# claudiotomasi/LearnMultigrid

Hardware: NVIDIA B200
Metric: vcycle_fine_grid_dof_per_s (higher is better)
Workload: dtype f64

## Files before the change

### include/mgb200.h

```cpp
#ifndef MGB200_H
#define MGB200_H

#include <stdint.h>

#ifdef __cplusplus
extern "C" {
#endif

typedef enum {
    MG_OK = 0,
    MG_ERR_INVALID = -1,
    MG_ERR_CUDA = -2,
    MG_ERR_UNSUPPORTED = -3,
    MG_ERR_OVERFLOW = -4,
    MG_ERR_SINGULAR = -5
} mg_status;

int mg_version(void);
const char *mg_last_error(void);
int64_t mg_struct_size(int which);
int mg_set_pdl(int enabled);
int mg_device_info(int *sm_count, int64_t *global_mem, int *cc);


// ... 11 lines not shown
int mg_gs_lex_sweep_csr(int64_t n, const int32_t *d_indptr, const int32_t *d_indices, const double *d_values,
                        double *d_x, const double *d_b, const int64_t *d_level_ptr,
                        const int32_t *d_level_rows, int64_t nlevels, int iterations, void *stream);
int mg_prolong_correct_csr(int64_t n, const int32_t *d_indptr, const int32_t *d_indices,
                           const double *d_values, const double *d_e, double *d_u, void *stream);

typedef struct {
    int64_t nrows;
    int64_t ncols;
    int64_t nslices;
    const int64_t *d_slice_ptr;
    const int32_t *d_cols;
    const double *d_vals;
    int64_t max_slice_len;
    int64_t uniform_len;
    const uint16_t *d_slice_rec;
    const int32_t *d_rec_table;
    int32_t nrec, n_spec;
    const int64_t *h_spec_row;
    const int32_t *h_spec_rec;
    const unsigned char *d_val_idx;
    const double *d_val_table;
    const double *d_rec_vals;
    const double *h_spec_vals;
} mg_sell;

int mg_sell_slice_offsets(const mg_sell *A, int32_t *d_off, int64_t *d_nregular, void *stream);
int64_t mg_value_dict_workspace(void);
int mg_value_dict_build(int64_t n, const double *d_vals, unsigned char *d_index, double *d_table, void *d_work,
                        int *h_count, void *stream);
int mg_set_value_dict(int enabled);
int mg_set_implied_values(int enabled);
int mg_set_implied_columns(int enabled);
int64_t mg_set_implied_min_rows(int64_t rows);
int mg_sell_spmv(const mg_sell *A, const double *d_x, double *d_y, void *stream);
int mg_sell_residual(const mg_sell *A, const double *d_x, const double *d_b, double *d_r, void *stream);
int mg_sell_residual_rows(const mg_sell *A, const double *d_x, const double *d_b, double *d_r, int64_t row0,
                          int64_t row1, void *stream);
int mg_sell_residual_norm2(const mg_sell *A, const double *d_x, const double *d_b, double *d_partials,
                           double *d_norm2, void *stream);
int64_t mg_norm_workspace_size(int64_t n);
int64_t mg_set_tma_min_rows(int64_t rows);
int64_t mg_set_wide_min_len(int64_t len);
int mg_set_short_rows_per_thread(int r);
int64_t mg_set_short_min_rows(int64_t rows);
int64_t mg_set_wide_max_rows(int64_t rows);
int mg_sell_jacobi(const mg_sell *A, const double *d_dinv, const double *d_x, const double *d_b,
                   double *d_x_out, double omega, void *stream);
int mg_sell_gs_rows(const mg_sell *A, double *d_x, const double *d_b, int64_t row0, int64_t row1,
                    void *stream);
int mg_sell_gs_rows_tail(const mg_sell *A, double *d_x, const double *d_b, int64_t row0, int64_t row1, int tail,
                         double *d_r, double *d_partials, int *h_nblocks, void *stream);
int mg_sell_gs_tail_ok(const mg_sell *A, int64_t row0, int64_t row1);
int mg_sell_gs_zero_first(int64_t n_vec, int64_t row0, int64_t row1, const double *d_diag, const double *d_b,
                          double *d_x, void *stream);
int mg_sell_prolong_correct(const mg_sell *Q, const double *d_e, const double *d_u, double *d_u_out,
                            void *stream);
int mg_sell_prolong_correct_rows(const mg_sell *Q, const double *d_e, const double *d_u, double *d_u_out, int64_t row0,
                                 int64_t row1, void *stream);

int mg_dot(int64_t n, const double *d_x, const double *d_y, double *d_partials, double *d_out, void *stream);
int mg_axpby(int64_t n, double a, const double *d_x, double b, const double *d_y, double *d_out, void *stream);
int mg_fill(int64_t n, double value, double *d_x, void *stream);
int mg_gather(int64_t n, const int32_t *d_idx, const double *d_in, double *d_out, void *stream);
int mg_scatter(int64_t n, const int32_t *d_idx, const double *d_in, double *d_out, void *stream);

// ... 270 lines not shown
```

### learnmultigrid_b200/_lib.py

```python
import ctypes
import os
import subprocess

_HERE = os.path.dirname(os.path.abspath(__file__))
LIB_PATH = os.path.join(_HERE, "libmgb200.so")
CSRC = os.path.join(_HERE, "csrc")

c_i32p = ctypes.c_void_p
c_f64p = ctypes.c_void_p
c_i64 = ctypes.c_int64
c_int = ctypes.c_int
c_dbl = ctypes.c_double
c_vp = ctypes.c_void_p

MG_SMOOTH_JACOBI, MG_SMOOTH_MCGS, MG_SMOOTH_LEXGS = 0, 1, 2
MG_COARSE_DENSE, MG_COARSE_BCR = 0, 1
MG_LEVEL_PROPER_COLORING, MG_LEVEL_NONZERO_DIAG = 1, 2
SLICE_IRREGULAR = -2 ** 31


class MgError(RuntimeError):
    pass


# ... 80 lines not shown
    "mg_device_info": (c_int, [ctypes.POINTER(c_int), ctypes.POINTER(c_i64), ctypes.POINTER(c_int)]),
    "mg_spmv_csr": (c_int, [c_i64, c_vp, c_vp, c_vp, c_vp, c_vp, c_vp]),
    "mg_residual_csr": (c_int, [c_i64, c_vp, c_vp, c_vp, c_vp, c_vp, c_vp, c_vp]),
    "mg_jacobi_sweep_csr": (c_int, [c_i64, c_vp, c_vp, c_vp, c_vp, c_vp, c_vp, c_vp, c_dbl, c_vp]),
    "mg_gs_multicolor_sweep_csr": (c_int, [c_i64, c_vp, c_vp, c_vp, c_vp, c_vp, ctypes.POINTER(c_i64), c_vp,
                                           c_int, c_vp]),
    "mg_gs_lex_sweep_csr": (c_int, [c_i64, c_vp, c_vp, c_vp, c_vp, c_vp, c_vp, c_vp, c_i64, c_int, c_vp]),
    "mg_prolong_correct_csr": (c_int, [c_i64, c_vp, c_vp, c_vp, c_vp, c_vp, c_vp]),
    "mg_sell_spmv": (c_int, [ctypes.POINTER(mg_sell), c_vp, c_vp, c_vp]),
    "mg_sell_slice_offsets": (c_int, [ctypes.POINTER(mg_sell), c_vp, c_vp, c_vp]),
    "mg_set_implied_min_rows": (c_i64, [c_i64]),
    "mg_tri_boxes_2d": (c_int, [c_i64, c_vp, c_vp, c_vp, c_vp, ctypes.c_int32, c_vp, c_vp, c_vp]),
    "mg_tri_incidence_2d": (c_int, [c_i64, c_vp, c_vp, c_vp, ctypes.c_int32, c_vp, c_vp, c_vp, c_vp]),
    "mg_tri_pairs_2d": (c_int, [c_i64, c_vp, c_vp, c_vp, c_vp, ctypes.c_int32, c_vp, c_vp, c_vp, c_vp, c_vp, c_vp, c_vp]),
    "mg_value_dict_workspace": (c_i64, []),
    "mg_value_dict_build": (c_int, [c_i64, c_vp, c_vp, c_vp, c_vp, ctypes.POINTER(c_int), c_vp]),
    "mg_set_value_dict": (c_int, [c_int]),
    "mg_set_implied_values": (c_int, [c_int]),
    "mg_set_short_rows_per_thread": (c_int, [c_int]),
    "mg_set_short_min_rows": (c_i64, [c_i64]),
    "mg_level_inspect": (c_int, [ctypes.POINTER(mg_sell), c_int, c_vp, c_vp, c_vp, c_vp]),
    "mg_sell_residual_rows": (c_int, [ctypes.POINTER(mg_sell), c_vp, c_vp, c_vp, c_i64, c_i64, c_vp]),
    "mg_sell_gs_rows_tail": (c_int, [ctypes.POINTER(mg_sell), c_vp, c_vp, c_i64, c_i64, c_int, c_vp, c_vp,
                                     ctypes.POINTER(c_int), c_vp]),
    "mg_sell_gs_tail_ok": (c_int, [ctypes.POINTER(mg_sell), c_i64, c_i64]),
    "mg_sell_gs_zero_first": (c_int, [c_i64, c_i64, c_i64, c_vp, c_vp, c_vp, c_vp]),
    "mg_sell_prolong_correct_rows": (c_int, [ctypes.POINTER(mg_sell), c_vp, c_vp, c_vp, c_i64, c_i64, c_vp]),
    "mg_vcycle_norm": (c_int, [ctypes.POINTER(mg_level), c_int, ctypes.POINTER(mg_cycle_params), c_vp, c_vp, c_vp]),
    "mg_set_cycle_fusion": (c_int, [c_int]),
    "mg_pcg_start": (c_int, [c_vp, ctypes.POINTER(mg_level), ctypes.POINTER(mg_pcg), c_vp]),
    "mg_pcg_iterate": (c_int, [c_vp, ctypes.POINTER(mg_level), c_int, ctypes.POINTER(mg_cycle_params),
                               ctypes.POINTER(mg_pcg), c_int, c_vp]),
    "mg_set_implied_columns": (c_int, [c_int]),
    "mg_sell_residual": (c_int, [ctypes.POINTER(mg_sell), c_vp, c_vp, c_vp, c_vp]),
    "mg_sell_residual_norm2": (c_int, [ctypes.POINTER(mg_sell), c_vp, c_vp, c_vp, c_vp, c_vp]),
    "mg_norm_workspace_size": (c_i64, [c_i64]),
    "mg_set_tma_min_rows": (c_i64, [c_i64]),
    "mg_sell_halo_mask": (c_int, [ctypes.POINTER(mg_sell), c_i64, c_vp, c_vp]),
    "mg_set_fused_exchange": (c_int, [c_int]),
    "mg_set_wide_min_len": (c_i64, [c_i64]),
    "mg_set_wide_max_rows": (c_i64, [c_i64]),
    "mg_sell_jacobi": (c_int, [ctypes.POINTER(mg_sell), c_vp, c_vp, c_vp, c_vp, c_dbl, c_vp]),
    "mg_sell_gs_rows": (c_int, [ctypes.POINTER(mg_sell), c_vp, c_vp, c_i64, c_i64, c_vp]),
    "mg_sell_prolong_correct": (c_int, [ctypes.POINTER(mg_sell), c_vp, c_vp, c_vp, c_vp]),
    "mg_dot": (c_int, [c_i64, c_vp, c_vp, c_vp, c_vp, c_vp]),
    "mg_axpby": (c_int, [c_i64, c_dbl, c_vp, c_dbl, c_vp, c_vp, c_vp]),
    "mg_fill": (c_int, [c_i64, c_dbl, c_vp, c_vp]),
    "mg_gather": (c_int, [c_i64, c_vp, c_vp, c_vp, c_vp]),
    "mg_scatter": (c_int, [c_i64, c_vp, c_vp, c_vp, c_vp]),
    "mg_dense_inverse": (c_int, [c_i64, c_vp, c_vp, c_vp, c_vp]),
    "mg_dense_inverse_workspace": (c_i64, [c_i64]),
    "mg_dense_gemv": (c_int, [c_i64, c_i64, c_vp, c_vp, c_vp, c_vp]),
    "mg_bcr_blocks_from_csr": (c_int, [c_i64, c_i64, c_i64, c_vp, c_vp, c_vp, c_vp, c_vp, c_vp, c_vp, c_vp]),
    "mg_dense_inverse_batched": (c_int, [c_i64, c_i64, c_vp, c_i64, c_vp, c_i64, c_vp, c_vp, c_vp]),
    "mg_dense_gemm_batched": (c_int, [c_i64, c_i64, c_vp, c_i64, c_vp, c_i64, c_vp, c_i64, c_dbl, c_dbl, c_vp]),
    "mg_bcr_solve": (c_int, [ctypes.POINTER(mg_bcr), c_vp, c_vp, c_vp]),
    "mg_bcr_solve_dist": (c_int, [ctypes.POINTER(mg_comm), ctypes.POINTER(mg_bcr), ctypes.POINTER(mg_bcr_dist), c_vp,
                                  c_vp, c_vp]),
    "mg_csr_to_dense": (c_int, [c_i64, c_vp, c_vp, c_vp, c_vp, c_vp]),
    "mg_scan_workspace_size": (c_i64, [c_i64]),
    "mg_exclusive_scan_i32": (c_int, [c_i64, c_vp, c_vp, c_vp, c_vp, c_i64, c_vp]),
    "mg_spgemm_symbolic": (c_int, [c_i64, c_vp, c_vp, c_vp, c_vp, c_int, c_int, c_vp, c_vp, c_vp]),
    "mg_spgemm_numeric": (c_int, [c_i64, c_vp, c_vp, c_vp, c_vp, c_vp, c_vp, c_int, c_int, c_vp, c_vp, c_vp, c_vp,
                                  c_vp, c_vp]),
    "mg_csr_compact_nonzeros": (c_int, [c_i64, c_vp, c_vp, c_vp, c_vp, c_vp, c_vp, c_vp]),
    "mg_sort_workspace_size": (c_i64, [c_i64]),
# ... 66 lines not shown
_testing_lib = None


def build(force=False, verbose=False):
    cmd = ["make", "-C", CSRC, "-j8"]
    if force:
        cmd.append("-B")
    out = subprocess.run(cmd, stdout=subprocess.PIPE, stderr=subprocess.STDOUT, text=True)
    if out.returncode != 0:
        raise MgError("building libmgb200.so failed:\n" + out.stdout)
    if verbose:
        print(out.stdout)
    return LIB_PATH


def load():
    global _lib
    if _lib is not None:
        return _lib
    if not os.path.exists(LIB_PATH):
        raise MgError("libmgb200.so is not built (%s); run `python -c 'import __graft_entry__ as g; g.build()'`"
                      % LIB_PATH)
    lib = ctypes.CDLL(LIB_PATH)
    for name, (res, args) in _SIGNATURES.items():
        fn = getattr(lib, name)
        fn.restype = res
        fn.argtypes = args
    if os.environ.get("MGB_PDL", "1") == "0":
        lib.mg_set_pdl(0)
    if os.environ.get("MGB_FUSED_EXCHANGE", "1") == "0":
        lib.mg_set_fused_exchange(0)
    if os.environ.get("MGB_IMPLIED_COLUMNS", "1") == "0":
        lib.mg_set_implied_columns(0)
    if "MGB_IMPLIED_MIN_ROWS" in os.environ:
        lib.mg_set_implied_min_rows(int(os.environ["MGB_IMPLIED_MIN_ROWS"]))
    if os.environ.get("MGB_VALUE_DICT", "1") == "0":
        lib.mg_set_value_dict(0)
    if os.environ.get("MGB_IMPLIED_VALUES", "1") == "0":
        lib.mg_set_implied_values(0)
    if "MGB_SHORT_ROWS" in os.environ:
        lib.mg_set_short_rows_per_thread(int(os.environ["MGB_SHORT_ROWS"]))
    if os.environ.get("MGB_CYCLE_FUSION", "1") == "0":
        lib.mg_set_cycle_fusion(0)
    if "MGB_WIDE_MIN_LEN" in os.environ:
        lib.mg_set_wide_min_len(int(os.environ["MGB_WIDE_MIN_LEN"]))
    if "MGB_WIDE_MAX_ROWS" in os.environ:
        lib.mg_set_wide_max_rows(int(os.environ["MGB_WIDE_MAX_ROWS"]))
    _lib = lib
    return lib


def load_testing():
    global _testing_lib
    if _testing_lib is not None:
        return _testing_lib
    path = os.path.join(os.path.dirname(LIB_PATH), "libmgb200_testing.so")
    if not os.path.exists(path):
        raise MgError("libmgb200_testing.so is not built (%s); run `python -c 'import __graft_entry__ as g; g.build()'`" % path)
    lib = ctypes.CDLL(path)
    for table in (_SIGNATURES, _TESTING_SIGNATURES):
        for name, (res, args) in table.items():
            fn = getattr(lib, name)
            fn.restype = res
            fn.argtypes = args
    _testing_lib = lib
    return lib
# ... 22 lines not shown
```

### learnmultigrid_b200/csrc/sell_core.cuh

```cuda
#pragma once
#include <type_traits>
#include "exchange.cuh"
#include "sell_api.cuh"

namespace mgb {

struct SellArgs {
    const int64_t *__restrict__ slice_ptr;
    const int32_t *__restrict__ cols;
    const double *__restrict__ vals;
    const unsigned short *__restrict__ slice_rec;
    const int32_t *__restrict__ rec_table;
    int32_t spec_id;
    int32_t spec_off[8];
    int32_t spec_lo, spec_hi;
    const double *__restrict__ rec_vals;
    double spec_val[8];
    double spec_diag;
    uint32_t spec_dmask;
    const unsigned char *__restrict__ vidx;
    const double *__restrict__ vtab;
    int64_t row_begin;
    int64_t row_end;
    int64_t first_row;
// ... 352 lines not shown
#pragma unroll
    for (int r = 0; r < R; ++r) {
#pragma unroll
        for (int j = 0; j < LEN; ++j)
            if (j < len[r]) {
                cc[r][j] = ld_stream(A.cols + base[r] + j * kSlice);
                if (VAL8) ii[r][j] = ld_stream(A.vidx + base[r] + j * kSlice);
                else vv[r][j] = ld_stream(A.vals + base[r] + j * kSlice);
            }
        av[r] = (MODE == PROLONG && act[r]) ? aux[row[r]] : 0.0;
    }
    if (VAL8) {
#pragma unroll
        for (int r = 0; r < R; ++r)
#pragma unroll
            for (int j = 0; j < LEN; ++j)
                if (j < len[r]) vv[r][j] = __ldg(A.vtab + ii[r][j]);
    }
#pragma unroll
    for (int r = 0; r < R; ++r)
#pragma unroll
        for (int j = 0; j < LEN; ++j)
            if (j < len[r]) xx[r][j] = x[cc[r][j]];
#pragma unroll
    for (int r = 0; r < R; ++r) {
        double sum = 0.0;
#pragma unroll
        for (int j = 0; j < LEN; ++j)
            if (j < len[r]) sum = mul_add_unfused(sum, vv[r][j], xx[r][j]);
        if (act[r]) y[row[r]] = MODE == PROLONG ? __dadd_rn(av[r], sum) : sum;
    }
}

__host__ __device__ constexpr int fused_min_ctas(int m, int len, bool uniform, bool impl) {
    if (mode_is_tail(m)) return (len <= 5 || (uniform && len <= 7)) ? 6 : 1;
    return mode_min_ctas(m, len, uniform, impl);
}

template <int MODE, int LEN, bool UNIFORM, bool IMPL, bool VAL8, bool IMPV = false>
__global__ void __launch_bounds__(kBlock, fused_min_ctas(MODE, LEN, UNIFORM, IMPL))
sell_kernel_fused(SellArgs A, const double *x, const double *__restrict__ b, const double *aux, double *y, double omega,
                  double *__restrict__ partials, const ExArgs fx, const unsigned char *__restrict__ mask) {
    pdl_prologue();
    const int nex = fx.npeers * fx.ctas_per_peer;
    if ((int)blockIdx.x < nex) {
        fused_exchange_cta(fx, (int)blockIdx.x);
        if (mode_has_partials(MODE)) {}
        return;
    }
    sell_body<MODE, LEN, UNIFORM, true, IMPL, VAL8, IMPV>(A, x, b, aux, y, omega, partials, (int64_t)blockIdx.x - nex, &fx, mask);
}

constexpr int kWideU = 5;
constexpr int kWideMaxLen = 64;

template <int MODE, int WPS>
__global__ void __launch_bounds__(kBlock)
sell_wide_kernel(SellArgs A, int uniform_len, const double *x, const double *__restrict__ b, const double *aux,
                 double *y, double omega, double *__restrict__ partials) {
    pdl_prologue();
    constexpr int SPC = kBlock / 32 / WPS;
    __shared__ double prod[SPC][kWideMaxLen][kSlice];
    __shared__ unsigned char skip[SPC][kWideMaxLen][kSlice];
    const int warp = threadIdx.x >> 5, lane = threadIdx.x & 31;
    const int sl = warp / WPS, w = warp % WPS;
    const int64_t slice = (A.first_row >> 5) + (int64_t)blockIdx.x * SPC + sl;
// ... 71 lines not shown
            const bool upd = diag != 0.0;
            double xn = 0.0;
            if (upd) {
                xn = __ddiv_rn(__dsub_rn(bv, sum), diag);
                y[row] = xn;
            }
            if (MODE != GS) {
                double s2 = 0.0;
                for (int k = 0; k < len; ++k) {
                    const double p = prod[sl][k][lane];
                    s2 = __dadd_rn(s2, skip[sl][k][lane] ? __dmul_rn(p, xn) : p);
                }
                const double r = __dsub_rn(bv, s2);
                if (MODE == GS_RES) A.r_out[row] = r;
                else contrib = r * r;
            }
        }
    }
    if (mode_has_partials(MODE)) {
        const double s = block_sum_last<kBlock>(contrib);
        if (threadIdx.x == 0) partials[blockIdx.x] = s;
    }
}

extern int64_t g_wide_min_len;
extern int64_t g_wide_max_rows;
extern int64_t g_tma_min_rows;
extern int g_implied_columns;
extern int64_t g_implied_min_rows;
extern int g_value_dict;
extern int g_implied_values;
extern int g_short_rows_per_thread;
extern int64_t g_short_min_rows;

template <int MODE>
int launch_sell_tma(const mg_sell *M, int64_t max_len, const double *x, const double *b, const double *aux, double *y,
                    double omega, double *partials, int64_t row0, int64_t row1, int *grid_out, cudaStream_t st,
                    const char *name);

inline bool sell_uses_wide(const mg_sell *A, int64_t row0, int64_t row1) {
    const int64_t ml = A->max_slice_len;
    return g_wide_min_len > 0 && ml >= g_wide_min_len && ml <= kWideMaxLen && row1 - row0 <= g_wide_max_rows;
}
bool sell_fusable(const mg_sell *A, int64_t row0, int64_t row1);
bool sell_gs_tail_ok(const mg_sell *A, int64_t row0, int64_t row1);

inline SellArgs sell_args(const mg_sell *A, int64_t row0, int64_t row1, double *r_out) {
    SellArgs a;
    a.slice_ptr = A->d_slice_ptr;
    a.cols = A->d_cols;
    a.vals = A->d_vals;
    a.slice_rec = A->d_slice_rec;
    a.rec_table = A->d_rec_table;
    a.spec_id = 0;
    for (int j = 0; j < 8; ++j) a.spec_off[j] = 0;
    a.spec_lo = 0;
    a.spec_hi = (int32_t)(A->ncols > 0 ? A->ncols - 1 : 0);
    a.vidx = A->d_val_idx;
    a.vtab = A->d_val_table;
    a.rec_vals = A->d_rec_vals;
    for (int j = 0; j < 8; ++j) a.spec_val[j] = 0.0;
    a.spec_diag = 0.0;
    a.spec_dmask = 0;
    a.row_begin = row0;
    a.row_end = row1;
    a.first_row = row0 & ~(int64_t)(kSlice - 1);
// ... 33 lines not shown
                    a.spec_val[j] = vj;
                    if (j < A->uniform_len && a.spec_off[j] == 0) {
                        unsigned long long b;
                        memcpy(&b, &vj, sizeof(b));
                        bits |= b;
                        if (vj != 0.0) a.spec_dmask |= 1u << j;
                    }
                }
                memcpy(&a.spec_diag, &bits, sizeof(bits));
            }
            return;
        }
}

template <int MODE>
static int launch_sell(const mg_sell *A, const double *x, const double *b, const double *aux, double *y,
                       double omega, double *partials, int64_t row0, int64_t row1, cudaStream_t st,
                       const char *name, int *nblocks_out = nullptr, const SellFuse *fuse = nullptr,
                       double *r_out = nullptr) {
    if (nblocks_out) *nblocks_out = 0;
    if (fuse && !sell_fusable(A, row0, row1)) return set_error(MG_ERR_INVALID, name, "this launch cannot carry an exchange site");
    if (row1 <= row0) return MG_OK;
    if (A->nrows > 0x7fffffffLL || A->ncols > 0x7fffffffLL) return set_error(MG_ERR_OVERFLOW, name, "2^31 rows or more");
    if (mode_is_tail(MODE) && !sell_gs_tail_ok(A, row0, row1)) return set_error(MG_ERR_INVALID, name, "rows too long for a sweep with a fused residual");
    if constexpr (MODE <= PROLONG) {
        if (g_tma_min_rows > 0 && row1 - row0 >= g_tma_min_rows && A->max_slice_len > 0) {
            int grid = 0;
            const int rc = launch_sell_tma<MODE>(A, A->max_slice_len, x, b, aux, y, omega, partials, row0, row1, &grid, st, name);
            if (rc <= 0) {
                if (nblocks_out) *nblocks_out = grid;
                return rc;
            }
        }
    }
    SellArgs a = sell_args(A, row0, row1, r_out);
    if (sell_use_implied(A, row0, row1)) sell_pick_spec(A, row0, a);
    const int64_t nthreads = row1 - a.first_row;
    const int64_t ml = A->max_slice_len;
    const bool uni = A->uniform_len > 0 && A->uniform_len == ml;
    if (sell_uses_wide(A, row0, row1)) {
        const int wps = ml <= 4 * kWideU ? 4 : 8;
        const int spc = kBlock / 32 / wps;
        const int64_t nsl = (nthreads + kSlice - 1) / kSlice;
        const int64_t wgrid = (nsl + spc - 1) / spc;
        if (wgrid > 0x7fffffffLL) return set_error(MG_ERR_OVERFLOW, name, "grid too large");
        if (wps == 4)
            launch_k(sell_wide_kernel<MODE, 4>, (unsigned)wgrid, kBlock, st, a, (int)(uni ? ml : 0), x, b, aux, y, omega, partials);
        else
            launch_k(sell_wide_kernel<MODE, 8>, (unsigned)wgrid, kBlock, st, a, (int)(uni ? ml : 0), x, b, aux, y, omega, partials);
        MG_CHECK_LAUNCH(name);
        if (nblocks_out) *nblocks_out = (int)wgrid;
        return MG_OK;
    }
    const int blk = fuse ? kBlock : kSellBlock;
    const int64_t grid = (nthreads + blk - 1) / blk;
    if (grid + (fuse ? fuse->nex : 0) > 0x7fffffffLL) return set_error(MG_ERR_OVERFLOW, name, "grid too large");
    if constexpr (MODE == SPMV || MODE == PROLONG) {
        if (!fuse && ml >= 1 && ml <= 2 && g_short_rows_per_thread > 1 && row1 - row0 >= g_short_min_rows && (uni || A->d_slice_ptr)) {
            const int R = g_short_rows_per_thread >= 4 ? 4 : 2;
            const unsigned sg = (unsigned)(((nthreads + kBlock - 1) / kBlock + R - 1) / R);
            const bool dict = sell_use_dict(A);
#define MG_SHORT(L, RR)                                                                                 \
    do {                                                                                                \
        if (dict && uni) launch_k(sell_short_kernel<MODE, L, RR, true, true>, sg, kBlock, st, a, x, aux, y);    \
        else if (dict) launch_k(sell_short_kernel<MODE, L, RR, true, false>, sg, kBlock, st, a, x, aux, y);    \
        else if (uni) launch_k(sell_short_kernel<MODE, L, RR, false, true>, sg, kBlock, st, a, x, aux, y);     \
// ... 58 lines not shown
```

### learnmultigrid_b200/csrc/sell_kernels.cu

```cuda
#include "sell_core.cuh"

namespace mgb {

int64_t g_wide_min_len = 9;
int64_t g_wide_max_rows = 1 << 18;
int64_t g_tma_min_rows = 0;
int g_implied_columns = 1;
int64_t g_implied_min_rows = 1 << 19;
int g_value_dict = 1;
int g_implied_values = 1;
int g_short_rows_per_thread = 2;
int64_t g_short_min_rows = 1 << 18;

__global__ void __launch_bounds__(kBlock)
sell_slice_offsets_kernel(int64_t nslices, int64_t nrows, int len, const int32_t *__restrict__ cols,
                          int32_t *__restrict__ off, unsigned long long *__restrict__ nregular) {
    const int64_t w = ((int64_t)blockIdx.x * kBlock + threadIdx.x) >> 5;
    const int lane = threadIdx.x & 31;
    if (w >= nslices) return;
    const int64_t row = w * kSlice + lane;
    bool regular = (w + 1) * kSlice <= nrows;
    for (int j = 0; j < kOffStride; ++j) {
        int64_t rel0 = 0;
        if (j < len) {
            const int64_t rel = (int64_t)cols[(w * len + j) * kSlice + lane] - row;
            rel0 = __shfl_sync(0xffffffffu, rel, 0);
            regular = __all_sync(0xffffffffu, rel == rel0) && regular;
        }
        if (lane == 0) off[w * kOffStride + j] = (int32_t)rel0;
    }
    if (lane == 0) {
        if (!regular) off[w * kOffStride] = kSliceIrregular;
        else if (nregular) atomicAdd(nregular, 1ull);
    }
}

__global__ void __launch_bounds__(kBlock)
sell_halo_mask_kernel(int64_t nslices, const int64_t *__restrict__ slice_ptr, int64_t uniform_len,
                      const int32_t *__restrict__ cols, int64_t first_halo_col, unsigned char *__restrict__ mask) {
    const int64_t s = ((int64_t)blockIdx.x * kBlock + threadIdx.x) >> 5;
    const int lane = threadIdx.x & 31;
    if (s >= nslices) return;
    const int64_t base = uniform_len > 0 ? s * kSlice * uniform_len : slice_ptr[s];
// ... 152 lines not shown
    const int64_t ns = A->nslices;
    sell_halo_mask_kernel<<<(unsigned)((ns * 32 + kBlock - 1) / kBlock), kBlock, 0, (cudaStream_t)stream>>>(
        ns, A->d_slice_ptr, A->uniform_len, A->d_cols, first_halo_col, d_mask);
    MG_CHECK_LAUNCH("sell_halo_mask");
    return MG_OK;
}
int mg_sell_slice_offsets(const mg_sell *A, int32_t *d_off, int64_t *d_nregular, void *stream) {
    if (int rc = check_sell(A)) return rc;
    MG_REQUIRE(d_off && A->uniform_len > 0 && A->uniform_len == A->max_slice_len && A->uniform_len <= kOffStride,
               "uniform SELL matrix with at most 8 entries per row expected");
    MG_REQUIRE(((uintptr_t)d_off & 31) == 0, "offset table must be 32-byte aligned");
    if (A->nslices == 0) return MG_OK;
    sell_slice_offsets_kernel<<<(unsigned)((A->nslices * 32 + kBlock - 1) / kBlock), kBlock, 0, (cudaStream_t)stream>>>(
        A->nslices, A->nrows, (int)A->uniform_len, A->d_cols, d_off, (unsigned long long *)d_nregular);
    MG_CHECK_LAUNCH("sell_slice_offsets");
    return MG_OK;
}
int mg_level_inspect(const mg_sell *A, int ncolors, const int64_t *d_color_ptr, double *d_diag, int32_t *d_flags,
                     void *stream) {
    if (int rc = check_sell(A)) return rc;
    MG_REQUIRE(d_flags && ncolors >= 0 && (ncolors == 0 || d_color_ptr), "null argument");
    if (A->nrows == 0) return MG_OK;
    sell_inspect_kernel<<<(unsigned)((A->nrows + kBlock - 1) / kBlock), kBlock, 0, (cudaStream_t)stream>>>(
        A->nrows, A->d_slice_ptr, A->uniform_len > 0 && A->uniform_len == A->max_slice_len ? A->uniform_len : 0, A->d_cols,
        A->d_vals, ncolors, d_color_ptr, d_diag, d_flags);
    MG_CHECK_LAUNCH("sell_inspect");
    return MG_OK;
}
int mg_set_implied_columns(int enabled) {
    const int prev = g_implied_columns;
    g_implied_columns = enabled ? 1 : 0;
    return prev;
}
int64_t mg_set_implied_min_rows(int64_t rows) {
    const int64_t prev = g_implied_min_rows;
    g_implied_min_rows = rows < 0 ? 0 : rows;
    return prev;
}
int mg_set_value_dict(int enabled) {
    const int prev = g_value_dict;
    g_value_dict = enabled ? 1 : 0;
    return prev;
}
int mg_set_implied_values(int enabled) {
    const int prev = g_implied_values;
    g_implied_values = enabled ? 1 : 0;
    return prev;
}
int mg_set_short_rows_per_thread(int r) {
    const int prev = g_short_rows_per_thread;
    g_short_rows_per_thread = r >= 4 ? 4 : r >= 2 ? 2 : 1;
    return prev;
}
int64_t mg_set_short_min_rows(int64_t rows) {
    const int64_t prev = g_short_min_rows;
    g_short_min_rows = rows < 0 ? 0 : rows;
    return prev;
}
int64_t mg_set_wide_min_len(int64_t len) {
    const int64_t prev = g_wide_min_len;
    g_wide_min_len = len < 0 ? 0 : len;
    return prev;
}
int64_t mg_set_wide_max_rows(int64_t rows) {
    const int64_t prev = g_wide_max_rows;
    g_wide_max_rows = rows < 0 ? 0 : rows;
// ... 56 lines not shown
```

### learnmultigrid_b200/engine.py

```python
import ctypes
import os

import numpy as np
import scipy.sparse as sp

from . import _lib
from . import formats as F
from . import setup_device as SD
from .coarse import build_coarse_solver

DENSE_COARSE_MAX = 4096


class DeviceSell:

    def __init__(self, torch, A_csr, device, sell=None):
        slice_ptr, cols, vals = F.csr_to_sell(A_csr) if sell is None else sell
        self.shape = A_csr.shape
        self.nnz = int(A_csr.nnz)
        self.padded = int(slice_ptr[-1])
        self.slice_ptr = torch.from_numpy(slice_ptr).to(device)
        self.cols = torch.from_numpy(cols).to(device)
        self.vals = torch.from_numpy(vals).to(device)
        d = np.diff(slice_ptr) // 32
        self.max_len = int(d.max()) if len(d) else 0
        self.uniform_len = self.max_len if len(d) and int(d.min()) == self.max_len else 0
        self.struct = _lib.mg_sell(self.shape[0], self.shape[1], (self.shape[0] + 31) // 32,
                                   self.slice_ptr.data_ptr(), self.cols.data_ptr(), self.vals.data_ptr(),
                                   self.max_len, self.uniform_len)
        self._attach_value_dict()
        self._attach_slice_offsets()

    VALUE_DICT_MIN_ROWS = 1 << 16

    def _attach_value_dict(self):
        self.val_idx = self.val_table = None
        self.distinct_values = None
        floor = int(os.environ.get("MGB_VALUE_DICT_MIN_ROWS", self.VALUE_DICT_MIN_ROWS))
        if (os.environ.get("MGB_VALUE_DICT", "1") == "0" or not 1 <= self.max_len <= 8 or self.shape[0] < floor
                or self.vals.numel() == 0):
            return
        import torch
        lib = _lib.load()
        dev = self.vals.device
        idx = torch.empty(self.vals.numel(), dtype=torch.uint8, device=dev)
        table = torch.zeros(256, dtype=torch.float64, device=dev)
        work = torch.empty(int(lib.mg_value_dict_workspace()), dtype=torch.uint8, device=dev)
        cnt = ctypes.c_int(0)
        _lib.check(lib.mg_value_dict_build(self.vals.numel(), self.vals.data_ptr(), idx.data_ptr(), table.data_ptr(),
                                           work.data_ptr(), ctypes.byref(cnt), _lib.stream_handle(torch)),
                   "mg_value_dict_build")
        if cnt.value > 0:
            self.distinct_values = int(cnt.value)
            self.val_idx, self.val_table = idx, table
            self.struct.d_val_idx = idx.data_ptr()
            self.struct.d_val_table = table.data_ptr()

    IMPLIED_MIN_ROWS = 1 << 19

    def _attach_slice_offsets(self):
        self.slice_rec = self.rec_table = self.rec_vals = None
        self.regular_slices = 0
        self._spec_keep = None
        floor = int(os.environ.get("MGB_IMPLIED_MIN_ROWS", self.IMPLIED_MIN_ROWS))
        if (os.environ.get("MGB_IMPLIED_COLUMNS", "1") == "0" or not 1 <= self.uniform_len <= 8
                or self.shape[0] < max(floor // 2, 1)):
            return
        import torch
        nsl = (self.shape[0] + 31) // 32
        dev = self.cols.device
        off = torch.empty(nsl * 8, dtype=torch.int32, device=dev)
        cnt = torch.zeros(1, dtype=torch.int64, device=dev)
        _lib.check(_lib.load().mg_sell_slice_offsets(ctypes.byref(self.struct), off.data_ptr(), cnt.data_ptr(),
                                                     _lib.stream_handle(torch)), "mg_sell_slice_offsets")
        self.regular_slices = int(cnt.item())
        if 2 * self.regular_slices < nsl:
            return
        with_values = self.val_idx is not None and os.environ.get("MGB_IMPLIED_VALUES", "1") != "0"
        ids, self.rec_table, self.rec_vals, self.regular_slices = F.slice_records(
            torch, off.view(nsl, 8), self.val_idx if with_values else None, self.val_table if with_values else None,
            self.uniform_len)
        self.slice_rec = ids
        self.struct.d_slice_rec = ids.data_ptr()
        self.struct.d_rec_table = self.rec_table.data_ptr()
        self.struct.nrec = int(self.rec_table.shape[0])
        if self.rec_vals is not None:
            self.struct.d_rec_vals = self.rec_vals.data_ptr()
        self.set_spec_blocks([0, self.shape[0]])

    @property
    def slice_off(self):
        if self.slice_rec is None:
            return None
        import torch
        out = torch.zeros(self.slice_rec.numel(), 8, dtype=torch.int32, device=self.slice_rec.device)
        reg = self.slice_rec >= 0
        out[reg] = self.rec_table[self.slice_rec[reg].long()]
        out[~reg, 0] = _lib.SLICE_IRREGULAR
        return out.reshape(-1)

    def set_spec_blocks(self, row_ptr):
        if self.slice_rec is None:
            return
        import torch
        row_ptr = [int(v) for v in row_ptr]
        nb = len(row_ptr) - 1
        table = self.rec_table.cpu().numpy()
        vals_table = None if self.rec_vals is None else self.rec_vals.cpu().numpy()
        rows = (ctypes.c_int64 * (nb + 1))(*row_ptr)
        rec = (ctypes.c_int32 * (9 * max(nb, 1)))()
        vals = (ctypes.c_double * (8 * max(nb, 1)))()
        for k in range(nb):
            s0, s1 = row_ptr[k] // 32, max((row_ptr[k + 1] + 31) // 32, row_ptr[k] // 32 + 1)
            ids = self.slice_rec[s0:s1]
            ids = ids[ids >= 0]
            best = int(torch.bincount(ids.long(), minlength=1).argmax().item()) if ids.numel() else 0
            rec[9 * k] = best
            for j in range(8):
                rec[9 * k + 1 + j] = int(table[best, j])
                if vals_table is not None:
                    vals[8 * k + j] = float(vals_table[best, j])
        self._spec_keep = (rows, rec, vals)
        self.struct.n_spec = nb
        self.struct.h_spec_row = ctypes.cast(rows, ctypes.POINTER(ctypes.c_int64))
        self.struct.h_spec_rec = ctypes.cast(rec, ctypes.POINTER(ctypes.c_int32))
        if vals_table is not None:
            self.struct.h_spec_vals = ctypes.cast(vals, ctypes.POINTER(ctypes.c_double))

    @classmethod
    def from_device(cls, shape, nnz, slice_ptr, cols, vals, max_len=0, uniform_len=0):
        self = cls.__new__(cls)
        self.shape = tuple(shape)
        self.nnz = int(nnz)
        self.padded = int(cols.numel())
        self.slice_ptr, self.cols, self.vals = slice_ptr, cols, vals
        self.max_len = int(max_len)
        self.uniform_len = int(uniform_len)
        self.struct = _lib.mg_sell(shape[0], shape[1], (shape[0] + 31) // 32,
                                   slice_ptr.data_ptr(), cols.data_ptr(), vals.data_ptr(), self.max_len,
                                   self.uniform_len)
        self._attach_value_dict()
        self._attach_slice_offsets()
        return self

    def bytes(self):
        return self.padded * 12 + self.slice_ptr.numel() * 8

    def stream_bytes(self):
        nsl = (self.shape[0] + 31) // 32
        vbytes = 1 if (self.val_idx is not None and os.environ.get("MGB_VALUE_DICT", "1") != "0") else 8
        if self.slice_rec is None or self.shape[0] < self.IMPLIED_MIN_ROWS or nsl == 0:
            return self.padded * (4 + vbytes) + (0 if self.uniform_len else self.slice_ptr.numel() * 8)
        per_slice = 32 * self.uniform_len
        irregular = nsl - self.regular_slices
        if self.rec_vals is not None and os.environ.get("MGB_IMPLIED_VALUES", "1") != "0" and vbytes == 1:
            return irregular * per_slice * (4 + vbytes) + 2 * nsl
        return self.padded * vbytes + irregular * per_slice * 4 + 2 * nsl


class Level:
    pass


def algorithmic_bytes_csr(nnz, n):
    return 12 * nnz + 4 * (n + 1)


class DeviceHierarchy:

    def __init__(self, A, Q_list, smoother="jacobi", colors=None, device=None, setup="device",
                 dense_coarse_max=DENSE_COARSE_MAX, keep_host=True):
        torch = _lib.require_cuda()
        self.torch = torch
        self.lib = _lib.load()
        self.device = torch.device("cuda", torch.cuda.current_device()) if device is None else torch.device(device)
        if smoother not in ("jacobi", "mcgs", "lexgs"):
            raise ValueError("unknown smoother %r" % (smoother,))
        self.smoother = smoother
        self.nlevels = len(Q_list) + 1
        if self.nlevels < 2:
            raise ValueError("need at least one transfer operator (levels >= 2)")
        self.keep_host = keep_host
# ... 89 lines not shown
            s = arr[l]
            s.n = lev.n
            s.d_x, s.d_b, s.d_r, s.d_tmp = (t.data_ptr() for t in (lev.x, lev.b, lev.r, lev.tmp))
            if getattr(lev, "dist_struct", None) is not None:
                s.dist = ctypes.pointer(lev.dist_struct)
            if l < L - 1:
                s.A, s.Q, s.QT = lev.A.struct, lev.Q.struct, lev.QT.struct
                s.d_dinv = lev.dinv.data_ptr()
                if lev.color_ptr is not None:
                    cp = (ctypes.c_int64 * len(lev.color_ptr))(*[int(v) for v in lev.color_ptr])
                    self._keep.append(cp)
                    s.ncolors = len(lev.color_ptr) - 1
                    s.h_color_ptr = ctypes.cast(cp, ctypes.POINTER(ctypes.c_int64))
                    s.flags = int(getattr(lev, "flags", 0))
                    if getattr(lev, "diag", None) is not None:
                        s.d_diag = lev.diag.data_ptr()
                if getattr(lev, "csr", None) is not None and getattr(lev, "lex_ptr", None) is not None:
                    s.d_csr_indptr, s.d_csr_indices, s.d_csr_values = (t.data_ptr() for t in lev.csr)
                    s.d_lex_level_ptr = lev.lex_ptr.data_ptr()
                    s.d_lex_level_rows = lev.lex_rows.data_ptr()
                    s.lex_nlevels = lev.lex_nlevels
            else:
                s.coarse_kind = lev.coarse_kind
                if lev.coarse_kind == _lib.MG_COARSE_DENSE:
                    s.d_coarse_inv = lev.coarse_inv.data_ptr()
                else:
                    s.coarse_bcr = lev.coarse_bcr
                    if getattr(lev, "coarse_bcr_dist", None) is not None:
                        s.coarse_bcr_dist = ctypes.pointer(lev.coarse_bcr_dist)
        self._level_structs = arr

    def _inspect_levels(self):
        torch, dev = self.torch, self.device
        flag = torch.zeros(1, dtype=torch.int32, device=dev)
        st = _lib.stream_handle(torch)
        for lev in self.levels:
            if getattr(lev, "A", None) is None or lev.color_ptr is None:
                continue
            lev.diag = torch.empty(lev.n, dtype=torch.float64, device=dev)
            lev.A.set_spec_blocks(lev.color_ptr)
            have = getattr(lev, "flags", None) is not None
            cp = torch.tensor([int(v) for v in lev.color_ptr], dtype=torch.int64, device=dev)
            flag.zero_()
            _lib.check(self.lib.mg_level_inspect(ctypes.byref(lev.A.struct), 0 if have else len(lev.color_ptr) - 1,
                                                 cp.data_ptr(), lev.diag.data_ptr(), flag.data_ptr(), st),
                       "mg_level_inspect")
            if not have:
                bad = int(flag.item())
                lev.flags = ((0 if bad & 1 else _lib.MG_LEVEL_PROPER_COLORING)
                             | (0 if bad & 2 else _lib.MG_LEVEL_NONZERO_DIAG))

    @property
    def _pinned(self):
        if self._pinned_buf is None:
            import time
            t0 = time.perf_counter()
            self._pinned_buf = self.torch.empty(self.n, dtype=self.torch.float64, pin_memory=True)
            self.pinned_alloc_s = time.perf_counter() - t0
        return self._pinned_buf

    def _to_level0(self, host_vec, dst):
        torch = self.torch
        evt = getattr(self, "_pin_evt", None)
        if evt is not None:
            evt.synchronize()
        self._to_level0_enqueue(host_vec, dst)
        if evt is None:
            evt = self._pin_evt = torch.cuda.Event()
        evt.record(torch.cuda.current_stream())

    def _to_level0_enqueue(self, host_vec, dst):
        torch = self.torch
        if isinstance(host_vec, torch.Tensor):
# ... 257 lines not shown
```

### learnmultigrid_b200/formats.py

```python
import ctypes

import numpy as np
import scipy.sparse as sp

from . import _lib

SLICE = 32


def solver_csr(A):
    if sp.isspmatrix_csr(A) and A.dtype == np.float64 and A.has_canonical_format:
        return canonical_csr(A)
    return canonical_csr(sp.csc_matrix(A))


def canonical_csr(A):
    if not sp.issparse(A):
        A = sp.csr_matrix(np.asarray(A, dtype=np.float64))
    A = sp.csr_matrix(A, dtype=np.float64)
    A.sum_duplicates()
    A.sort_indices()
    if A.nnz >= 2 ** 31 or max(A.shape) >= 2 ** 31:
        raise OverflowError("matrix does not fit the int32 index contract")
    A.indptr = A.indptr.astype(np.int32, copy=False)
# ... 183 lines not shown
    n = A.shape[0]
    T = sp.csr_matrix((np.ones(A.nnz), A.indices, A.indptr), shape=A.shape).T.tocsr()
    T.sort_indices()
    tip, tix = T.indptr.astype(np.int32), T.indices.astype(np.int32)
    lib = _lib.load_testing()
    colors = np.empty(max(n, 1), dtype=np.int32)
    work = np.zeros(int(lib.mg_color_workspace_size(n)), dtype=np.uint8)
    rounds = ctypes.c_int64(0)
    rc = lib.mg_host_color_rounds(n, A.indptr.ctypes.data, A.indices.ctypes.data, tip.ctypes.data, tix.ctypes.data,
                                  colors.ctypes.data, work.ctypes.data, ctypes.byref(rounds))
    if rc:
        _lib.check(rc, "mg_host_color_rounds")
    colors = colors[:n]
    return colors, (int(colors.max()) + 1 if n else 0), int(rounds.value)


SLICE_IRREGULAR = -2 ** 31


def sell_slice_offsets(sell, nrows, length):
    slice_ptr, cols, _ = sell
    nsl = len(slice_ptr) - 1
    off = np.full((nsl, max(length, 1)), SLICE_IRREGULAR, dtype=np.int32)
    if nsl == 0 or length <= 0:
        return off
    c = np.asarray(cols, dtype=np.int64).reshape(nsl, length, SLICE)
    rows = (np.arange(nsl, dtype=np.int64) * SLICE)[:, None, None] + np.arange(SLICE, dtype=np.int64)[None, None, :]
    rel = c - rows
    regular = np.all(rel == rel[:, :, :1], axis=(1, 2)) & ((np.arange(nsl) + 1) * SLICE <= nrows)
    off[regular] = rel[regular][:, :, 0].astype(np.int32)
    return off


def slice_records(torch, off, val_idx=None, val_table=None, uniform_len=0, max_records=32766):
    nsl = int(off.shape[0])
    dev = off.device
    regular = off[:, 0] != SLICE_IRREGULAR
    n_regular = int(regular.sum().item())
    vrec = None
    if val_idx is not None and val_table is not None and uniform_len >= 1 and val_idx.numel() == nsl * 32 * uniform_len:
        v = val_idx.view(nsl, uniform_len, 32)
        same = (v == v[:, :, :1]).all(dim=2).all(dim=1)
        full = regular & same
        if n_regular > 0 and 10 * int(full.sum().item()) >= 9 * n_regular:
            vrec = torch.zeros(nsl, 8, dtype=torch.int32, device=dev)
            vrec[:, :uniform_len] = v[:, :, 0].to(torch.int32)
            regular = full
        del v, same, full
    keys = off if vrec is None else torch.cat([off, vrec], dim=1)
    recs, inverse, counts = torch.unique(keys[regular], dim=0, return_inverse=True, return_counts=True)
    order = torch.argsort(counts, descending=True)[:max_records]
    rank_of = torch.full((recs.shape[0],), -1, dtype=torch.int64, device=dev)
    rank_of[order] = torch.arange(order.numel(), device=dev)
    ids = torch.full((nsl,), -1, dtype=torch.int16, device=dev)
    ids[regular] = rank_of[inverse].to(torch.int16)
    rec_table = recs[order][:, :8].contiguous().to(torch.int32)
    rec_vals = None if vrec is None else val_table[recs[order][:, 8:16].long()].contiguous()
    return ids, rec_table, rec_vals, int((ids >= 0).sum().item())
```

Baseline: 29.44 billion.

## Compress transfer-operator slices into shared column/value pattern records

Rectangular transfer operators (restriction/prolongation) with uniform slice length are analysed on the GPU to find repeated per-slice patterns of column offsets and values. Matching slices are stored as a 16-bit record id plus a base column, and a new pattern kernel rebuilds columns and values from a small cached table instead of streaming them. The goal is to cut the memory traffic of SpMV and prolongation in the V-cycle. The cost is extra setup hashing and verification, and a fallback per-slice path for irregular slices inside the kernel.

```diff
diff --git a/include/mgb200.h b/include/mgb200.h
--- a/include/mgb200.h
+++ b/include/mgb200.h
@@ -67,6 +67,7 @@
 int mg_set_value_dict(int enabled);
 int mg_set_implied_values(int enabled);
 int mg_set_implied_columns(int enabled);
+int mg_set_implied_transfers(int enabled);
 int64_t mg_set_implied_min_rows(int64_t rows);
 int mg_sell_spmv(const mg_sell *A, const double *d_x, double *d_y, void *stream);
 int mg_sell_residual(const mg_sell *A, const double *d_x, const double *d_b, double *d_r, void *stream);
diff --git a/learnmultigrid_b200/_lib.py b/learnmultigrid_b200/_lib.py
--- a/learnmultigrid_b200/_lib.py
+++ b/learnmultigrid_b200/_lib.py
@@ -136,6 +136,7 @@
     "mg_pcg_iterate": (c_int, [c_vp, ctypes.POINTER(mg_level), c_int, ctypes.POINTER(mg_cycle_params),
                                ctypes.POINTER(mg_pcg), c_int, c_vp]),
     "mg_set_implied_columns": (c_int, [c_int]),
+    "mg_set_implied_transfers": (c_int, [c_int]),
     "mg_sell_residual": (c_int, [ctypes.POINTER(mg_sell), c_vp, c_vp, c_vp, c_vp]),
     "mg_sell_residual_norm2": (c_int, [ctypes.POINTER(mg_sell), c_vp, c_vp, c_vp, c_vp, c_vp]),
     "mg_norm_workspace_size": (c_i64, [c_i64]),
@@ -268,6 +269,8 @@
         lib.mg_set_fused_exchange(0)
     if os.environ.get("MGB_IMPLIED_COLUMNS", "1") == "0":
         lib.mg_set_implied_columns(0)
+    if os.environ.get("MGB_IMPLIED_TRANSFERS", "1") == "0":
+        lib.mg_set_implied_transfers(0)
     if "MGB_IMPLIED_MIN_ROWS" in os.environ:
         lib.mg_set_implied_min_rows(int(os.environ["MGB_IMPLIED_MIN_ROWS"]))
     if os.environ.get("MGB_VALUE_DICT", "1") == "0":
diff --git a/learnmultigrid_b200/csrc/sell_core.cuh b/learnmultigrid_b200/csrc/sell_core.cuh
--- a/learnmultigrid_b200/csrc/sell_core.cuh
+++ b/learnmultigrid_b200/csrc/sell_core.cuh
@@ -408,6 +408,100 @@
     }
 }
 
+constexpr int kPatBlocks = 8;
+
+struct PatArgs {
+    const unsigned short *__restrict__ rec;
+    const int32_t *__restrict__ base;
+    const int32_t *__restrict__ delta;
+    const double *__restrict__ pvals;
+    const int32_t *__restrict__ cols;
+    const double *__restrict__ vals;
+    int32_t spec_row[kPatBlocks];
+    int32_t spec_id[kPatBlocks];
+    int32_t row_begin, row_end, first_row;
+    uint32_t col_max;
+};
+
+template <int MODE, int LEN, int R, bool SPEC>
+__global__ void __launch_bounds__(kBlock, LEN >= 8 ? 4 : 5)
+sell_pattern_kernel(PatArgs A, const double *x, const double *aux, double *y) {
+    static_assert(MODE == SPMV || MODE == PROLONG, "slice patterns: SpMV and prolongation only");
+    pdl_prologue();
+    const int lane = threadIdx.x & 31;
+    int32_t row[R], bs[R], cc[R][LEN];
+    unsigned id[R];
+    bool in[R];
+    double vv[R][LEN], xx[R][LEN], av[R];
+#pragma unroll
+    for (int r = 0; r < R; ++r) {
+        row[r] = A.first_row + ((int32_t)blockIdx.x * R + r) * kBlock + (int32_t)threadIdx.x;
+        in[r] = row[r] < A.row_end;
+        bs[r] = in[r] ? __ldg(A.base + (row[r] >> 5)) : 0;
+        id[r] = in[r] ? ld_const_u16(A.rec + (row[r] >> 5)) : 0u;
+    }
+    int spec[R];
+    if (SPEC) {
+#pragma unroll
+        for (int r = 0; r < R; ++r) {
+            spec[r] = A.spec_id[0];
+#pragma unroll
+            for (int k = 1; k < kPatBlocks; ++k) spec[r] = row[r] >= A.spec_row[k] ? A.spec_id[k] : spec[r];
+#pragma unroll
+            for (int j = 0; j < LEN; ++j) cc[r][j] = __ldg(A.delta + (spec[r] * LEN + j) * kSlice + lane);
+        }
+    }
+#pragma unroll
+    for (int r = 0; r < R; ++r) av[r] = (MODE == PROLONG && in[r] && row[r] >= A.row_begin) ? aux[row[r]] : 0.0;
+    if (SPEC) {
+#pragma unroll
+        for (int r = 0; r < R; ++r)
+            if (in[r]) {
+#pragma unroll
+                for (int j = 0; j < LEN; ++j)
+                    xx[r][j] = ld_gather(x, (int32_t)min((uint32_t)(bs[r] + cc[r][j]), A.col_max));
+            }
+    }
+    bool redo[R];
+#pragma unroll
+    for (int r = 0; r < R; ++r) {
+        redo[r] = in[r] && (!SPEC || id[r] != (unsigned)spec[r]);
+        if (!in[r]) continue;
+        if (SPEC && !redo[r]) {
+#pragma unroll
+            for (int j = 0; j < LEN; ++j) vv[r][j] = __ldg(A.pvals + (spec[r] * LEN + j) * kSlice + lane);
+        } else if (id[r] == (unsigned)kRecIrregular) {
+            const int64_t ent = (int64_t)(row[r] >> 5) * (kSlice * LEN) + lane;
+#pragma unroll
+            for (int j = 0; j < LEN; ++j) {
+                cc[r][j] = ld_stream(A.cols + ent + j * kSlice);
+                vv[r][j] = ld_stream(A.vals + ent + j * kSlice);
+            }
+        } else {
+            const int o = (int)id[r] * LEN * kSlice + lane;
+#pragma unroll
+            for (int j = 0; j < LEN; ++j) {
+                cc[r][j] = bs[r] + __ldg(A.delta + o + j * kSlice);
+                vv[r][j] = __ldg(A.pvals + o + j * kSlice);
+            }
+        }
+    }
+#pragma unroll
+    for (int r = 0; r < R; ++r)
+        if (redo[r]) {
+#pragma unroll
+            for (int j = 0; j < LEN; ++j) xx[r][j] = ld_gather(x, cc[r][j]);
+        }
+#pragma unroll
+    for (int r = 0; r < R; ++r) {
+        if (!in[r] || row[r] < A.row_begin) continue;
+        double sum = 0.0;
+#pragma unroll
+        for (int j = 0; j < LEN; ++j) sum = mul_add_unfused(sum, vv[r][j], xx[r][j]);
+        y[row[r]] = MODE == PROLONG ? __dadd_rn(av[r], sum) : sum;
+    }
+}
+
 __host__ __device__ constexpr int fused_min_ctas(int m, int len, bool uniform, bool impl) {
     if (mode_is_tail(m)) return (len <= 5 || (uniform && len <= 7)) ? 6 : 1;
     return mode_min_ctas(m, len, uniform, impl);
@@ -545,6 +639,66 @@
 extern int g_implied_values;
 extern int g_short_rows_per_thread;
 extern int64_t g_short_min_rows;
+extern int g_implied_transfers;
+
+inline bool sell_use_patterns(const mg_sell *A, int64_t row0, int64_t row1) {
+    const int64_t ml = A->max_slice_len;
+    return g_implied_transfers && A->d_slice_rec && A->d_rec_table && A->d_rec_vals && A->nrec < 0 &&
+           A->uniform_len == ml && ml >= 1 && ml <= 8 && row1 - row0 >= g_implied_min_rows;
+}
+
+template <int MODE>
+int launch_sell_pattern(const mg_sell *A, const double *x, const double *aux, double *y, int64_t row0, int64_t row1,
+                        cudaStream_t st, const char *name, int *nblocks_out) {
+    const int L = (int)A->max_slice_len;
+    PatArgs a;
+    a.rec = A->d_slice_rec;
+    a.delta = A->d_rec_table;
+    a.base = A->d_rec_table + (int64_t)(-A->nrec) * L * kSlice;
+    a.pvals = A->d_rec_vals;
+    a.cols = A->d_cols;
+    a.vals = A->d_vals;
+    for (int k = 0; k < kPatBlocks; ++k) {
+        a.spec_row[k] = k == 0 ? 0 : INT32_MAX;
+        a.spec_id[k] = 0;
+    }
+    bool spec = false;
+    if (A->h_spec_row && A->h_spec_rec && A->n_spec > 0) {
+        spec = true;
+        for (int k = 0; k < A->n_spec; ++k) {
+            if (k < kPatBlocks) {
+                a.spec_row[k] = k == 0 ? 0 : (int32_t)A->h_spec_row[k];
+                a.spec_id[k] = A->h_spec_rec[9 * k];
+            }
+            if (A->h_spec_row[k] < row1 && A->h_spec_row[k + 1] > row0 && A->h_spec_rec[9 * k + 1] < 500) spec = false;
+        }
+    }
+    a.row_begin = (int32_t)row0;
+    a.row_end = (int32_t)row1;
+    a.first_row = (int32_t)(row0 & ~(int64_t)(kSlice - 1));
+    a.col_max = (uint32_t)(A->ncols > 0 ? A->ncols - 1 : 0);
+    const int R = L <= 2 ? 2 : 1;
+    const unsigned grid = (unsigned)(((row1 - a.first_row + kBlock - 1) / kBlock + R - 1) / R);
+#define MG_PAT(LL, RR)                                                                                          \
+    do {                                                                                                        \
+        if (spec) launch_k(sell_pattern_kernel<MODE, LL, RR, true>, grid, kBlock, st, a, x, aux, y);            \
+        else launch_k(sell_pattern_kernel<MODE, LL, RR, false>, grid, kBlock, st, a, x, aux, y);                \
+    } while (0)
+    switch (L) {
+        case 1: MG_PAT(1, 2); break;
+        case 2: MG_PAT(2, 2); break;
+        case 3: MG_PAT(3, 1); break;
+        case 4: MG_PAT(4, 1); break;
+        case 5: MG_PAT(5, 1); break;
+        case 6: MG_PAT(6, 1); break;
+        case 7: MG_PAT(7, 1); break;
+        default: MG_PAT(8, 1); break;
+    }
+#undef MG_PAT
+    MG_CHECK_LAUNCH(name);
+    if (nblocks_out) *nblocks_out = (int)grid;
+    return MG_OK;
+}
 
 template <int MODE>
 int launch_sell_tma(const mg_sell *M, int64_t max_len, const double *x, const double *b, const double *aux, double *y,
@@ -644,6 +798,9 @@
                 return rc;
             }
         }
+    }
+    if constexpr (MODE == SPMV || MODE == PROLONG) {
+        if (!fuse && sell_use_patterns(A, row0, row1)) return launch_sell_pattern<MODE>(A, x, aux, y, row0, row1, st, name, nblocks_out);
     }
     SellArgs a = sell_args(A, row0, row1, r_out);
     if (sell_use_implied(A, row0, row1)) sell_pick_spec(A, row0, a);
diff --git a/learnmultigrid_b200/csrc/sell_kernels.cu b/learnmultigrid_b200/csrc/sell_kernels.cu
--- a/learnmultigrid_b200/csrc/sell_kernels.cu
+++ b/learnmultigrid_b200/csrc/sell_kernels.cu
@@ -9,6 +9,7 @@
 int64_t g_implied_min_rows = 1 << 19;
 int g_value_dict = 1;
 int g_implied_values = 1;
+int g_implied_transfers = 1;
 int g_short_rows_per_thread = 2;
 int64_t g_short_min_rows = 1 << 18;
 
@@ -227,6 +228,11 @@
     g_implied_columns = enabled ? 1 : 0;
     return prev;
 }
+int mg_set_implied_transfers(int enabled) {
+    const int prev = g_implied_transfers;
+    if (enabled >= 0) g_implied_transfers = enabled ? 1 : 0;
+    return prev;
+}
 int64_t mg_set_implied_min_rows(int64_t rows) {
     const int64_t prev = g_implied_min_rows;
     g_implied_min_rows = rows < 0 ? 0 : rows;
diff --git a/learnmultigrid_b200/engine.py b/learnmultigrid_b200/engine.py
--- a/learnmultigrid_b200/engine.py
+++ b/learnmultigrid_b200/engine.py
@@ -30,6 +30,7 @@
                                    self.max_len, self.uniform_len)
         self._attach_value_dict()
         self._attach_slice_offsets()
+        self._attach_patterns()
 
     VALUE_DICT_MIN_ROWS = 1 << 16
 
@@ -87,6 +88,58 @@
         if self.rec_vals is not None:
             self.struct.d_rec_vals = self.rec_vals.data_ptr()
         self.set_spec_blocks([0, self.shape[0]])
+
+    PATTERN_SAMPLE = 4096
+
+    def _attach_patterns(self):
+        self.pat_rec = self.pat_table = self.pat_vals = None
+        self.pattern_slices = 0
+        floor = int(os.environ.get("MGB_IMPLIED_MIN_ROWS", self.IMPLIED_MIN_ROWS))
+        L = self.uniform_len
+        if (os.environ.get("MGB_IMPLIED_TRANSFERS", "1") == "0" or self.slice_rec is not None
+                or self.shape[0] == self.shape[1] or not 1 <= L <= 8 or self.shape[0] < max(floor, 1)):
+            return
+        import torch
+        nsl = (self.shape[0] + 31) // 32
+        if nsl > 2 * self.PATTERN_SAMPLE:
+            pick = torch.linspace(0, nsl - 2, self.PATTERN_SAMPLE, device=self.cols.device).long()
+            sc = self.cols.view(nsl, 32 * L)[pick].reshape(-1)
+            sv = self.vals.view(nsl, 32 * L)[pick].reshape(-1)
+            *_, nreg = F.pattern_records(torch, sc, sv, self.PATTERN_SAMPLE * 32, L)
+            if 2 * nreg < self.PATTERN_SAMPLE:
+                return
+        base, ids, delta, pvals, nreg = F.pattern_records(torch, self.cols, self.vals, self.shape[0], L)
+        if 2 * nreg < nsl:
+            return
+        self.pat_rec, self.pat_vals = ids, pvals
+        self.pat_table = torch.cat([delta.reshape(-1), base])
+        self.pattern_slices = nreg
+        s = self.struct
+        s.d_slice_rec, s.d_rec_table, s.d_rec_vals = ids.data_ptr(), self.pat_table.data_ptr(), pvals.data_ptr()
+        s.nrec = -int(delta.shape[0])
+        self.set_pattern_blocks([0, self.shape[0]])
+
+    def set_pattern_blocks(self, row_ptr):
+        if self.pat_rec is None:
+            return
+        import torch
+        row_ptr = [int(v) for v in row_ptr]
+        if len(row_ptr) > 9:
+            row_ptr = row_ptr[:8] + row_ptr[-1:]
+        nb = len(row_ptr) - 1
+        rows = (ctypes.c_int64 * (nb + 1))(*row_ptr)
+        rec = (ctypes.c_int32 * (9 * max(nb, 1)))()
+        for k in range(nb):
+            ids = self.pat_rec[row_ptr[k] // 32:max((row_ptr[k + 1] + 31) // 32, row_ptr[k] // 32 + 1)]
+            n = ids.numel()
+            ids = ids[ids >= 0]
+            cnt = torch.bincount(ids.long(), minlength=1) if ids.numel() else torch.zeros(1, dtype=torch.int64)
+            rec[9 * k] = int(cnt.argmax().item())
+            rec[9 * k + 1] = int(1000 * int(cnt.max().item()) // max(n, 1))
+        self._spec_keep = (rows, rec)
+        self.struct.n_spec = nb
+        self.struct.h_spec_row = ctypes.cast(rows, ctypes.POINTER(ctypes.c_int64))
+        self.struct.h_spec_rec = ctypes.cast(rec, ctypes.POINTER(ctypes.c_int32))
 
     @property
     def slice_off(self):
@@ -141,6 +194,7 @@
                                    self.uniform_len)
         self._attach_value_dict()
         self._attach_slice_offsets()
+        self._attach_patterns()
         return self
 
     def bytes(self):
@@ -148,6 +202,8 @@
 
     def stream_bytes(self):
         nsl = (self.shape[0] + 31) // 32
+        if self.pat_rec is not None and _lib.load().mg_set_implied_transfers(-1):
+            return (nsl - self.pattern_slices) * 32 * self.uniform_len * 12 + 6 * nsl
         vbytes = 1 if (self.val_idx is not None and os.environ.get("MGB_VALUE_DICT", "1") != "0") else 8
         if self.slice_rec is None or self.shape[0] < self.IMPLIED_MIN_ROWS or nsl == 0:
             return self.padded * (4 + vbytes) + (0 if self.uniform_len else self.slice_ptr.numel() * 8)
@@ -303,6 +359,9 @@
 
     def _inspect_levels(self):
         torch, dev = self.torch, self.device
+        for lev, nxt in zip(self.levels[:-1], self.levels[1:]):
+            if getattr(lev, "QT", None) is not None and getattr(nxt, "color_ptr", None) is not None:
+                lev.QT.set_pattern_blocks(nxt.color_ptr)
         flag = torch.zeros(1, dtype=torch.int32, device=dev)
         st = _lib.stream_handle(torch)
         for lev in self.levels:
@@ -310,6 +369,8 @@
                 continue
             lev.diag = torch.empty(lev.n, dtype=torch.float64, device=dev)
             lev.A.set_spec_blocks(lev.color_ptr)
+            if getattr(lev, "Q", None) is not None:
+                lev.Q.set_pattern_blocks(lev.color_ptr)
             have = getattr(lev, "flags", None) is not None
             cp = torch.tensor([int(v) for v in lev.color_ptr], dtype=torch.int64, device=dev)
             flag.zero_()
diff --git a/learnmultigrid_b200/formats.py b/learnmultigrid_b200/formats.py
--- a/learnmultigrid_b200/formats.py
+++ b/learnmultigrid_b200/formats.py
@@ -239,6 +239,56 @@
     return off
 
 
+def sell_slice_patterns(sell, nrows, length):
+    slice_ptr, cols, vals = sell
+    nsl = len(slice_ptr) - 1
+    c = np.asarray(cols, dtype=np.int64).reshape(nsl, length, SLICE)
+    base = c[:, 0, 0].copy() if nsl else np.zeros(0, dtype=np.int64)
+    delta = c - base[:, None, None]
+    full = (np.arange(nsl) + 1) * SLICE <= nrows
+    return base, delta, np.asarray(vals, dtype=np.float64).reshape(nsl, length, SLICE), full
+
+
+def pattern_records(torch, cols, vals, nrows, length, max_records=256, min_slices=2, chunk=1 << 16):
+    dev = cols.device
+    nsl = int(cols.numel()) // (32 * length)
+    K = 32 * length
+    c = cols.view(nsl, K)
+    base = c[:, 0].contiguous()
+    vbits = vals.view(nsl, K).view(torch.int64)
+    gen = torch.Generator().manual_seed(20251)
+    w = torch.randint(1, 1 << 20, (2, 3, K), generator=gen, dtype=torch.int64).to(dev)
+
+    def pattern(s):
+        d = c[s].to(torch.int64) - base[s].to(torch.int64)[:, None]
+        v = vbits[s]
+        return torch.cat([d, v >> 32, v & 0xffffffff], dim=1)
+
+    keys = torch.empty(nsl, 2, dtype=torch.int64, device=dev)
+    for s0 in range(0, nsl, chunk):
+        s = slice(s0, min(s0 + chunk, nsl))
+        p = pattern(s)
+        keys[s, 0] = (p * w[0].reshape(1, -1)).sum(dim=1)
+        keys[s, 1] = (p * w[1].reshape(1, -1)).sum(dim=1)
+    _, inverse, counts = torch.unique(keys, dim=0, return_inverse=True, return_counts=True)
+    first = torch.full((counts.numel(),), nsl, dtype=torch.int64, device=dev)
+    first.scatter_reduce_(0, inverse, torch.arange(nsl, device=dev), reduce="amin")
+    ok = (torch.arange(nsl, device=dev) + 1) * 32 <= nrows
+    for s0 in range(0, nsl, chunk):
+        s = slice(s0, min(s0 + chunk, nsl))
+        ok[s] &= (pattern(s) == pattern(first[inverse[s]])).all(dim=1)
+    counts = torch.bincount(inverse[ok], minlength=counts.numel())
+    order = torch.argsort(counts, descending=True, stable=True)
+    order = order[counts[order] >= min_slices][:max_records]
+    rank_of = torch.full((counts.numel(),), -1, dtype=torch.int64, device=dev)
+    rank_of[order] = torch.arange(order.numel(), device=dev)
+    ids = torch.where(ok, rank_of[inverse], torch.full_like(inverse, -1)).to(torch.int16)
+    rep = first[order]
+    delta = (c[rep].to(torch.int64) - base[rep, None].to(torch.int64)).to(torch.int32).view(-1, length, 32).contiguous()
+    rvals = vals.view(nsl, K)[rep].view(-1, length, 32).contiguous()
+    return base.to(torch.int32), ids, delta, rvals, int((ids >= 0).sum().item())
+
+
 def slice_records(torch, off, val_idx=None, val_table=None, uniform_len=0, max_records=32766):
     nsl = int(off.shape[0])
     dev = off.device
```

New measurement: 31.03 billion, median of 6. 5.4% higher.
